# nrsyed/pytorch-yolov3

Hardware: AMD Instinct MI355X
Metric: frames/sec (608x608) (higher is better)
Workload: dtype bf16

## Files before the change

### pytorch-yolov3_amd/csrc/conv_fused.hip

```cpp
#include "common.h"
#include <type_traits>

namespace {

constexpr int kTO = 16;
constexpr int kSR = 2 * kTO + 1;
constexpr int kIR = kSR + 2;
constexpr int kInPitch = 144;
constexpr int kStemPitch = 80;
constexpr int kW1Pitch = 608;
constexpr int kNStem = kSR * kSR;
constexpr int kNFrag = (kNStem + 15) / 16;
constexpr int kThreads = 512;
constexpr int kInBytes = kIR * kInPitch * 2;
constexpr int kPatchElems = kIR * kIR * 3;
constexpr int kPre = (kPatchElems + kThreads - 1) / kThreads;
constexpr int kLds = 2 * kInBytes + kNStem * kStemPitch + 64 * kW1Pitch + 512;

template <typename T>
struct FusedArgs {
  const unsigned char *in;
  int H, W, batch;
  const T *w0;
  const float *sc0, *bi0;
  uint32_t flags0;
  const T *w1;
  int k_ld1;
  const float *sc1, *bi1;
  uint32_t flags1;
  T *out;
  int out_ld, Ho, Wo;
  int tiles_x, tiles_y, n_tiles;
  int dbg;
};

template <typename T>
__device__ __forceinline__ u32x2 bn_leaky_pack4(const f32x4 &a, const f32x4 &sc, const f32x4 &bi) {
  const f32x2 lo = f32x2{a[0], a[1]} * f32x2{sc[0], sc[1]} + f32x2{bi[0], bi[1]};
  const f32x2 hi = f32x2{a[2], a[3]} * f32x2{sc[2], sc[3]} + f32x2{bi[2], bi[3]};
  const f32x2 tl = lo * Y3_LEAKY_SLOPE, th = hi * Y3_LEAKY_SLOPE;
  return y3_pack4<T>(y3_vmax(lo[0], tl[0]), y3_vmax(lo[1], tl[1]), y3_vmax(hi[0], th[0]), y3_vmax(hi[1], th[1]));
}

template <typename T>
__global__ __launch_bounds__(kThreads) void conv_stem_s2_fused_kernel(FusedArgs<T> p) {
  typedef typename H16<T>::v8 V8;
  extern __shared__ __attribute__((aligned(16))) char smem[];
  T *in_tile = reinterpret_cast<T *>(smem);
  char *stem = smem + 2 * kInBytes;
  char *w1s = stem + kNStem * kStemPitch;
  T *lut = reinterpret_cast<T *>(w1s + 64 * kW1Pitch);

  const int tid = threadIdx.x, lane = tid & 63;
  const int wave = __builtin_amdgcn_readfirstlane(tid >> 6);
  const int fr = lane & 15, fq = lane >> 4;

  for (int i = tid; i < 64 * 36; i += kThreads) {
    const int co = i / 36, ch = i - co * 36;
    *reinterpret_cast<u32x4 *>(w1s + co * kW1Pitch + ch * 16) =
        *reinterpret_cast<const u32x4 *>(reinterpret_cast<const char *>(p.w1) + ((long long)co * p.k_ld1) * 2 + ch * 16);
  }
  V8 w0a[2], w0b[2];
#pragma unroll
  for (int st = 0; st < 2; ++st)
#pragma unroll
    for (int j = 0; j < 8; ++j) {
      const int k = st * 32 + fq * 8 + j;
      const int ky = k / 12, rem = k - ky * 12, kx = rem >> 2, c = rem & 3;
      const bool live = k < 36 && c < 3;
      const int kold = live ? ky * 9 + kx * 3 + c : 0;
      const T za = p.w0[(0 + fr) * 32 + kold], zb = p.w0[(16 + fr) * 32 + kold];
      w0a[st][j] = live ? za : (T)0.f;
      w0b[st][j] = live ? zb : (T)0.f;
    }
  int off_lo, off_hi;
  {
    const int k0 = fq * 8, k1 = fq * 8 + 4;
    off_lo = (k0 / 12) * kInPitch + (k0 % 12);
    off_hi = (k1 / 12) * kInPitch + (k1 % 12);
  }
  const int off_s1 = 2 * kInPitch + 8;
  const int cq = fq * 4;
  f32x4 sc0[2], bi0[2];
#pragma unroll
  for (int ni = 0; ni < 2; ++ni) {
    sc0[ni] = *reinterpret_cast<const f32x4 *>(p.sc0 + ni * 16 + cq);
    bi0[ni] = *reinterpret_cast<const f32x4 *>(p.bi0 + ni * 16 + cq);
  }

  int pr_row[kPre], pr_col[kPre], pr_dst[kPre];
  uint32_t pr_goff[kPre];
#pragma unroll
  for (int j = 0; j < kPre; ++j) {
    const int i = tid + j * kThreads;
    const int r = i / (kIR * 3), cb = i - r * (kIR * 3);
    pr_row[j] = r;
    pr_col[j] = cb;
    pr_goff[j] = (uint32_t)(r * p.W * 3 + cb);
    pr_dst[j] = r * kInPitch + (cb / 3) * 4 + (cb % 3);
  }
  const bool pr_last_live = tid + (kPre - 1) * kThreads < kPatchElems;
  auto tile_coords = [&](int tile, int &tx, int &ty, int &b) {
    int t = tile;
    tx = t % p.tiles_x;
    t /= p.tiles_x;
    ty = t % p.tiles_y;
    b = t / p.tiles_y;
  };
  auto patch_fetch = [&](int tile, unsigned char (&pre)[kPre]) {
    int tx, ty, b;
    tile_coords(tile, tx, ty, b);
    const int iy0 = 2 * ty * kTO - 2, ixb0 = (2 * tx * kTO - 2) * 3;
    const bool interior = iy0 >= 0 && iy0 + kIR <= p.H && ixb0 >= 0 && ixb0 + kIR * 3 <= p.W * 3;
    if (interior) {
      const unsigned char *base = p.in + ((long long)b * p.H + iy0) * p.W * 3 + ixb0;
#pragma unroll
      for (int j = 0; j < kPre; ++j) pre[j] = (j < kPre - 1 || pr_last_live) ? base[pr_goff[j]] : (unsigned char)0;
    } else {
#pragma unroll
      for (int j = 0; j < kPre; ++j) {
        const int iy = iy0 + pr_row[j], ixb = ixb0 + pr_col[j];
        unsigned char v = 0;
        if ((j < kPre - 1 || pr_last_live) && (unsigned)iy < (unsigned)p.H && ixb >= 0 && ixb < p.W * 3)
          v = p.in[((long long)b * p.H + iy) * p.W * 3 + ixb];
        pre[j] = v;
      }
    }
  };
  auto patch_store = [&](int buf, const unsigned char (&pre)[kPre]) {
    T *dst = in_tile + buf * (kIR * kInPitch);
#pragma unroll
    for (int j = 0; j < kPre; ++j)
      if (j < kPre - 1 || pr_last_live) dst[pr_dst[j]] = lut[pre[j]];
  };

  for (int i = tid; i < 2 * kIR * kInPitch / 2; i += kThreads) reinterpret_cast<uint32_t *>(in_tile)[i] = 0u;
  if (tid < 256) lut[tid] = (T)((float)tid / 255.0f);
  __syncthreads();
  int tile = blockIdx.x;
  int buf = 0;
  if (tile < p.n_tiles) {
    unsigned char pre[kPre];
    patch_fetch(tile, pre);
    patch_store(0, pre);
  }
  for (; tile < p.n_tiles; tile += gridDim.x) {
    int tx, ty, b;
    tile_coords(tile, tx, ty, b);
    const int oy0 = ty * kTO, ox0 = tx * kTO;
    __syncthreads();

    const T *patch = in_tile + buf * (kIR * kInPitch);
    const bool stem_inside = 2 * oy0 - 1 >= 0 && 2 * oy0 - 1 + kSR <= p.H && 2 * ox0 - 1 >= 0 && 2 * ox0 - 1 + kSR <= p.W;
    constexpr int kFG = 3;
    constexpr int kFragIters = (kNFrag + kThreads / 64 - 1) / (kThreads / 64);
    static_assert(kFragIters % kFG == 0, "fragment groups");
#pragma unroll 1
    for (int g = 0; g < ((p.dbg & 1) ? 0 : kFragIters); g += kFG) {
      u32x2 lo[kFG], hi[kFG], s1[kFG];
      int qv[kFG], syv[kFG], sxv[kFG];
#pragma unroll
      for (int j = 0; j < kFG; ++j) {
        const int q = (wave + (g + j) * (kThreads / 64)) * 16 + fr;
        const int qc = q < kNStem ? q : kNStem - 1;
        const int sy = qc / kSR, sx = qc - sy * kSR;
        const T *base = patch + sy * kInPitch + sx * 4;
        lo[j] = *reinterpret_cast<const u32x2 *>(base + off_lo);
        hi[j] = *reinterpret_cast<const u32x2 *>(base + off_hi);
        s1[j] = *reinterpret_cast<const u32x2 *>(base + off_s1);
        qv[j] = q;
        syv[j] = sy;
        sxv[j] = sx;
      }
      f32x4 acc0[kFG], acc1[kFG];
#pragma unroll
      for (int j = 0; j < kFG; ++j) {
        const V8 xf0 = __builtin_bit_cast(V8, u32x4{lo[j][0], lo[j][1], hi[j][0], hi[j][1]});
        acc0[j] = H16<T>::mfma(w0a[0], xf0, f32x4{0.f, 0.f, 0.f, 0.f});
        acc1[j] = H16<T>::mfma(w0b[0], xf0, f32x4{0.f, 0.f, 0.f, 0.f});
      }
#pragma unroll
      for (int j = 0; j < kFG; ++j) {
        const V8 xf1 = __builtin_bit_cast(V8, fq == 0 ? u32x4{s1[j][0], s1[j][1], 0u, 0u} : u32x4{0u, 0u, 0u, 0u});
        acc0[j] = H16<T>::mfma(w0a[1], xf1, acc0[j]);
        acc1[j] = H16<T>::mfma(w0b[1], xf1, acc1[j]);
      }
#pragma unroll
      for (int j = 0; j < kFG; ++j) {
        if (qv[j] < kNStem) {
          bool inside = true;
          if (!stem_inside) {
            const int gy = 2 * oy0 - 1 + syv[j], gx = 2 * ox0 - 1 + sxv[j];
            inside = (unsigned)gy < (unsigned)p.H && (unsigned)gx < (unsigned)p.W;
          }
#pragma unroll
          for (int ni = 0; ni < 2; ++ni) {
            u32x2 o = bn_leaky_pack4<T>(ni ? acc1[j] : acc0[j], sc0[ni], bi0[ni]);
            if (!inside) o = u32x2{0u, 0u};
            *reinterpret_cast<u32x2 *>(stem + qv[j] * kStemPitch + (ni * 16 + cq) * 2) = o;
          }
        }
      }
    }
    const int next_tile = tile + gridDim.x;
    unsigned char pre[kPre];
    if (next_tile < p.n_tiles && !(p.dbg & 8)) patch_fetch(next_tile, pre);
    __syncthreads();

    f32x4 acc[2][4];
#pragma unroll
    for (int mi = 0; mi < 2; ++mi)
#pragma unroll
      for (int nf = 0; nf < 4; ++nf) acc[mi][nf] = f32x4{0.f, 0.f, 0.f, 0.f};
#pragma unroll
    for (int tap = 0; tap < ((p.dbg & 2) ? 0 : 9); ++tap) {
      const int ky = tap / 3, kx = tap - ky * 3;
      u32x4 xf[2], wf[4];
#pragma unroll
      for (int mi = 0; mi < 2; ++mi) {
        const int q = (2 * (2 * wave + mi) + ky) * kSR + 2 * fr + kx;
        xf[mi] = *reinterpret_cast<const u32x4 *>(stem + q * kStemPitch + fq * 16);
      }
#pragma unroll
      for (int nf = 0; nf < 4; ++nf)
        wf[nf] = *reinterpret_cast<const u32x4 *>(w1s + (nf * 16 + fr) * kW1Pitch + tap * 64 + fq * 16);
#pragma unroll
      for (int mi = 0; mi < 2; ++mi)
#pragma unroll
        for (int nf = 0; nf < 4; ++nf)
          acc[mi][nf] = H16<T>::mfma(__builtin_bit_cast(V8, wf[nf]),
                                                                __builtin_bit_cast(V8, xf[mi]), acc[mi][nf]);
    }
    if (next_tile < p.n_tiles) patch_store(buf ^ 1, pre);
    __syncthreads();

#pragma unroll
    for (int nf = 0; nf < 4; ++nf) {
      const f32x4 s1 = *reinterpret_cast<const f32x4 *>(p.sc1 + nf * 16 + cq);
      const f32x4 b1 = *reinterpret_cast<const f32x4 *>(p.bi1 + nf * 16 + cq);
#pragma unroll
      for (int mi = 0; mi < 2; ++mi) {
        const int px = (2 * wave + mi) * kTO + fr;
        const int co = nf * 16 + cq;
        *reinterpret_cast<u32x2 *>(stem + px * 128 + (((co >> 3) ^ (px & 7)) << 4) + (co & 7) * 2) =
            bn_leaky_pack4<T>(acc[mi][nf], s1, b1);
      }
    }
    __syncthreads();
#pragma unroll
    for (int j = 0; j < kTO * kTO * 8 / kThreads; ++j) {
      const int i = tid + j * kThreads;
      const int px = i >> 3, ch = i & 7;
      const int oy = oy0 + (px >> 4), ox = ox0 + (px & 15);
      if (oy < p.Ho && ox < p.Wo && !(p.dbg & 4)) {
        const u32x4 v = *reinterpret_cast<const u32x4 *>(stem + px * 128 + ((ch ^ (px & 7)) << 4));
        *reinterpret_cast<u32x4 *>(p.out + (((long long)b * p.Ho + oy) * p.Wo + ox) * p.out_ld + ch * 8) = v;
      }
    }
    buf ^= 1;
  }
}


constexpr int kPX = 16, kPY = 8;
constexpr int kPSX = 2 * kPX + 1;
constexpr int kPSY = 2 * kPY + 1;
constexpr int kPIX = kPSX + 2, kPIY = kPSY + 2;
constexpr int kPNStem = kPSX * kPSY;
constexpr int kPNFrag = (kPNStem + 15) / 16;
constexpr int kPInBytes = kPIY * kInPitch * 2;
constexpr int kPStemBytes = kPNStem * kStemPitch;
constexpr int kPStage = 8 * 16 * 128;
constexpr int kPLds = 2 * kPInBytes + 2 * kPStemBytes + 64 * kW1Pitch + 512 + kPStage;
static_assert(kPLds <= 160 * 1024, "LDS budget");
static_assert(kPX == 16 && kPY == 8, "one 16-pixel output row per conv wave");

template <typename T, int NC>
__global__ __launch_bounds__(1024) void conv_stem_s2_ws_kernel(FusedArgs<T> p) {
  typedef typename H16<T>::v8 V8;
  constexpr int NS = 16 - NC, NT = 1024;
  constexpr int MR = kPY / NC;
  constexpr int kIters = (kPNFrag + NS - 1) / NS;
  constexpr int kPairs = kPIY * ((kPIX * 3 + 1) / 2);
  constexpr int kPre = (kPairs + 64 * NS - 1) / (64 * NS);
  extern __shared__ __attribute__((aligned(16))) char smem[];
  char *in_tile = smem;
  char *stem0 = smem + 2 * kPInBytes;
  char *w1s = stem0 + 2 * kPStemBytes;
  T *lut = reinterpret_cast<T *>(w1s + 64 * kW1Pitch);
  char *stage = reinterpret_cast<char *>(lut) + 512;

  const int tid = threadIdx.x, lane = tid & 63;
  const int wave = __builtin_amdgcn_readfirstlane(tid >> 6);
  const int fr = lane & 15, fq = lane >> 4;
  const bool is_stem = wave >= NC;

  for (int i = tid; i < 64 * 36; i += NT) {
    const int j = i / 36, ch = i - j * 36;
    const int co = y3_pair_perm(j);
    *reinterpret_cast<u32x4 *>(w1s + j * kW1Pitch + ch * 16) =
        *reinterpret_cast<const u32x4 *>(reinterpret_cast<const char *>(p.w1) + ((long long)co * p.k_ld1) * 2 + ch * 16);
  }
  for (int i = tid; i < 2 * kPInBytes / 4; i += NT) reinterpret_cast<uint32_t *>(in_tile)[i] = 0u;
  if (tid < 256) lut[tid] = (T)((float)tid / 255.0f);
  __syncthreads();
  const int tile0 = blockIdx.x, stride = gridDim.x;
  if (tile0 >= p.n_tiles) return;
  struct TilePos { int tile, tx, ty, b; };
  auto pos_of = [&](int tile) {
    TilePos t;
    t.tile = tile;
    t.tx = tile % p.tiles_x;
    const int r = tile / p.tiles_x;
    t.ty = r % p.tiles_y;
    t.b = r / p.tiles_y;
    return t;
  };
  const TilePos dpos = pos_of(stride);
  auto advance = [&](TilePos &t) {
    t.tile += stride;
    t.tx += dpos.tx;
    int c = t.tx >= p.tiles_x ? 1 : 0;
    t.tx -= c ? p.tiles_x : 0;
    t.ty += dpos.ty + c;
    c = t.ty >= p.tiles_y ? 1 : 0;
    t.ty -= c ? p.tiles_y : 0;
    t.b += dpos.b + c;
  };

  if (is_stem) {
    const int sw = wave - NC, stid = tid - 64 * NC;
    V8 w0a[2], w0b[2];
#pragma unroll
    for (int st = 0; st < 2; ++st)
#pragma unroll
      for (int j = 0; j < 8; ++j) {
        const int k = st * 32 + fq * 8 + j;
        const int ky = k / 12, rem = k - ky * 12, kx = rem >> 2, c = rem & 3;
        const bool live = k < 36 && c < 3;
        const int kold = live ? ky * 9 + kx * 3 + c : 0;
        const T za = p.w0[y3_pair_perm(fr) * 32 + kold], zb = p.w0[y3_pair_perm(16 + fr) * 32 + kold];
        w0a[st][j] = live ? za : (T)0.f;
        w0b[st][j] = live ? zb : (T)0.f;
      }
    int off_lo, off_hi;
    {
      const int k0 = fq * 8, k1 = fq * 8 + 4;
      off_lo = ((k0 / 12) * kInPitch + (k0 % 12)) * 2;
      off_hi = ((k1 / 12) * kInPitch + (k1 % 12)) * 2;
    }
    constexpr int off_s1 = (2 * kInPitch + 8) * 2;
    f32x4 sc0[2], bi0[2];
#pragma unroll
    for (int ni = 0; ni < 2; ++ni) {
      sc0[ni] = *reinterpret_cast<const f32x4 *>(p.sc0 + fq * 8 + ni * 4);
      bi0[ni] = *reinterpret_cast<const f32x4 *>(p.bi0 + fq * 8 + ni * 4);
    }
    int fr_patch[kIters];
    uint32_t fr_live = 0;
#pragma unroll
    for (int j = 0; j < kIters; ++j) {
      const int q = (sw + NS * j) * 16 + fr;
      const int qc = q < kPNStem ? q : kPNStem - 1;
      const int sy = qc / kPSX, sx = qc - sy * kPSX;
      fr_patch[j] = (sy * kInPitch + sx * 4) * 2;
      fr_live |= (q < kPNStem ? 1u : 0u) << j;
    }
    int stem_wr = ((sw * 16 + fr) * kStemPitch) + fq * 16;
    asm volatile("" : "+v"(stem_wr));
    constexpr int kRowPairs = (kPIX * 3 + 1) / 2;
    int pr_dst[kPre];
    uint32_t pr_goff[kPre];
    uint32_t pr_one = 0;
#pragma unroll
    for (int j = 0; j < kPre; ++j) {
      const int i = stid + j * 64 * NS;
      const int r = i / kRowPairs, cb = 2 * (i - r * kRowPairs);
      pr_goff[j] = (uint32_t)(r * p.W * 3 + cb);
      pr_dst[j] = (r * kInPitch + (cb / 3) * 4 + (cb % 3)) * 2 | (cb % 3 == 2 ? 1 : 0);
      pr_one |= (cb + 1 >= kPIX * 3 ? 1u : 0u) << j;
    }
    const bool pr_last_live = stid + (kPre - 1) * 64 * NS < kPairs;
    const bool pairs_aligned = ((p.W * 3) & 1) == 0 && (reinterpret_cast<size_t>(p.in) & 1) == 0;
    auto patch_fetch = [&](const TilePos &t, unsigned short (&pre)[kPre]) {
      const int tx = t.tx, ty = t.ty, b = t.b;
      const int iy0 = 2 * ty * kPY - 2, ixb0 = (2 * tx * kPX - 2) * 3;
      const bool interior = pairs_aligned && iy0 >= 0 && iy0 + kPIY <= p.H && ixb0 >= 0 && ixb0 + 2 * kRowPairs <= p.W * 3;
      if (interior) {
        const unsigned char *base = p.in + ((long long)b * p.H + iy0) * p.W * 3 + ixb0;
#pragma unroll
        for (int j = 0; j < kPre; ++j)
          pre[j] = (j < kPre - 1 || pr_last_live) ? *reinterpret_cast<const unsigned short *>(base + pr_goff[j]) : (unsigned short)0;
      } else {
#pragma unroll
        for (int j = 0; j < kPre; ++j) {
          const int i = stid + j * 64 * NS;
          const int r = i / kRowPairs, cb = 2 * (i - r * kRowPairs);
          const int iy = iy0 + r, ixb = ixb0 + cb;
          unsigned int v = 0;
          if ((j < kPre - 1 || pr_last_live) && (unsigned)iy < (unsigned)p.H) {
            const unsigned char *row = p.in + ((long long)b * p.H + iy) * p.W * 3;
            if (ixb >= 0 && ixb < p.W * 3) v = row[ixb];
            if (ixb + 1 >= 0 && ixb + 1 < p.W * 3 && cb + 1 < kPIX * 3) v |= (unsigned int)row[ixb + 1] << 8;
          }
          pre[j] = (unsigned short)v;
        }
      }
    };
    auto patch_store = [&](int buf, const unsigned short (&pre)[kPre]) {
      char *dst = in_tile + buf * kPInBytes;
#pragma unroll
      for (int j = 0; j < kPre; ++j)
        if (j < kPre - 1 || pr_last_live) {
          char *d = dst + (pr_dst[j] & ~1);
          *reinterpret_cast<T *>(d) = lut[pre[j] & 255];
          if (!((pr_one >> j) & 1u)) *reinterpret_cast<T *>(d + 2 + 2 * (pr_dst[j] & 1)) = lut[pre[j] >> 8];
        }
    };
    auto stem_image = [&](const char *patch, char *img, const TilePos &t) {
      const int oy0 = t.ty * kPY, ox0 = t.tx * kPX;
      const bool all_inside = 2 * oy0 - 1 >= 0 && 2 * oy0 - 1 + kPSY <= p.H && 2 * ox0 - 1 >= 0 && 2 * ox0 - 1 + kPSX <= p.W;
      auto group = [&](auto g0, auto cnt) {
        constexpr int g = decltype(g0)::value, G = decltype(cnt)::value;
        u32x2 lo[G], hi[G], s1[G];
#pragma unroll
        for (int j = 0; j < G; ++j) {
          const char *base = patch + fr_patch[g + j];
          lo[j] = *reinterpret_cast<const u32x2 *>(base + off_lo);
          hi[j] = *reinterpret_cast<const u32x2 *>(base + off_hi);
          s1[j] = *reinterpret_cast<const u32x2 *>(base + off_s1);
        }
        f32x4 a0[G], a1[G];
#pragma unroll
        for (int j = 0; j < G; ++j) {
          const V8 xf0 = __builtin_bit_cast(V8, u32x4{lo[j][0], lo[j][1], hi[j][0], hi[j][1]});
          a0[j] = H16<T>::mfma(w0a[0], xf0, f32x4{0.f, 0.f, 0.f, 0.f});
          a1[j] = H16<T>::mfma(w0b[0], xf0, f32x4{0.f, 0.f, 0.f, 0.f});
        }
#pragma unroll
        for (int j = 0; j < G; ++j) {
          const V8 xf1 = __builtin_bit_cast(V8, u32x4{s1[j][0], s1[j][1], s1[j][0], s1[j][1]});
          a0[j] = H16<T>::mfma(w0a[1], xf1, a0[j]);
          a1[j] = H16<T>::mfma(w0b[1], xf1, a1[j]);
        }
#pragma unroll
        for (int j = 0; j < G; ++j) {
          u32x2 o0 = bn_leaky_pack4<T>(a0[j], sc0[0], bi0[0]);
          u32x2 o1 = bn_leaky_pack4<T>(a1[j], sc0[1], bi0[1]);
          if (!all_inside) {
            const int q = (sw + NS * (g + j)) * 16 + fr;
            const int qc = q < kPNStem ? q : kPNStem - 1;
            const int sy = qc / kPSX, sx = qc - sy * kPSX;
            const int gy = 2 * oy0 - 1 + sy, gx = 2 * ox0 - 1 + sx;
            if (!((unsigned)gy < (unsigned)p.H && (unsigned)gx < (unsigned)p.W)) {
              o0 = u32x2{0u, 0u};
              o1 = u32x2{0u, 0u};
            }
          }
          if ((fr_live >> (g + j)) & 1u) {
            char *dst = img + stem_wr + (g + j) * (NS * 16 * kStemPitch);
            *reinterpret_cast<u32x4 *>(dst) = u32x4{o0[0], o0[1], o1[0], o1[1]};
          }
        }
      };
      using std::integral_constant;
      static_assert(kIters == 5 || kIters == 3, "fragment groups");
      group(integral_constant<int, 0>{}, integral_constant<int, 3>{});
      if constexpr (kIters == 5) group(integral_constant<int, 3>{}, integral_constant<int, 2>{});
    };

    unsigned short pre[4][kPre];
    TilePos fpos = pos_of(tile0);
    TilePos ipos = fpos;
    {
      patch_fetch(fpos, pre[0]);
      patch_store(0, pre[0]);
      advance(fpos);
      if (fpos.tile < p.n_tiles) {
        patch_fetch(fpos, pre[1]);
        patch_store(1, pre[1]);
      }
      advance(fpos);
    }
    __builtin_amdgcn_s_waitcnt(0xC07F);
    __builtin_amdgcn_s_barrier();
#pragma unroll
    for (int k = 0; k < 3; ++k) {
      if (fpos.tile < p.n_tiles) patch_fetch(fpos, pre[k]);
      advance(fpos);
    }
    stem_image(in_tile, stem0, ipos);
    advance(ipos);
    __builtin_amdgcn_s_waitcnt(0xC07F);
    __builtin_amdgcn_s_barrier();
    int par = 0;
    Y3_STAMP_DECL
    auto step = [&](auto setc) {
      constexpr int set = decltype(setc)::value;
      if (fpos.tile < p.n_tiles) patch_fetch(fpos, pre[(set + 3) & 3]);
      advance(fpos);
      Y3_STAMP(0);
      const bool more = ipos.tile < p.n_tiles;
      if (more) stem_image(in_tile + (par ^ 1) * kPInBytes, stem0 + (par ^ 1) * kPStemBytes, ipos);
      advance(ipos);
      __builtin_amdgcn_s_waitcnt(0xC07F);
      Y3_STAMP(1);
      if (ipos.tile < p.n_tiles) patch_store(par, pre[set]);
      __builtin_amdgcn_s_waitcnt(0xC07F);
      Y3_STAMP(2);
      __builtin_amdgcn_s_barrier();
      Y3_STAMP(3);
      par ^= 1;
      return more;
    };
    using std::integral_constant;
    for (;;) {
      if (!step(integral_constant<int, 0>{})) break;
      if (!step(integral_constant<int, 1>{})) break;
      if (!step(integral_constant<int, 2>{})) break;
      if (!step(integral_constant<int, 3>{})) break;
    }
#ifdef Y3_STAMPS
    if (tid == 64 * NC) for (int _i = 0; _i < 4; ++_i) atomicAdd(&g_y3_stamps[_i], _st_acc[_i]);
#endif
    return;
  }

  const int a_rd = ((2 * wave * MR) * kPSX + 2 * fr) * kStemPitch + fq * 16;
  const int b_rd = fr * kW1Pitch + fq * 16;
  char *my_stage = stage + wave * (MR * 16 * 128);
  f32x4 s1v[4], b1v[4];
#pragma unroll
  for (int nf = 0; nf < 4; ++nf) {
    s1v[nf] = *reinterpret_cast<const f32x4 *>(p.sc1 + (nf >> 1) * 32 + fq * 8 + (nf & 1) * 4);
    b1v[nf] = *reinterpret_cast<const f32x4 *>(p.bi1 + (nf >> 1) * 32 + fq * 8 + (nf & 1) * 4);
  }
  __builtin_amdgcn_s_waitcnt(0xC07F);
  __builtin_amdgcn_s_barrier();
  __builtin_amdgcn_s_barrier();
  uint32_t st_off[2];
#pragma unroll
  for (int k = 0; k < 2; ++k) st_off[k] = (uint32_t)((((lane >> 3) + 8 * k) * p.out_ld + (lane & 7) * 8) * 2);
  int par = 0;
  Y3_STAMP_DECL
  for (TilePos pos = pos_of(tile0); pos.tile < p.n_tiles; advance(pos)) {
    const int b = pos.b;
    const int oy0 = pos.ty * kPY, ox0 = pos.tx * kPX;
    const char *img = stem0 + par * kPStemBytes;
    f32x4 acc[MR][4];
#pragma unroll
    for (int mr = 0; mr < MR; ++mr)
#pragma unroll
      for (int nf = 0; nf < 4; ++nf) acc[mr][nf] = f32x4{0.f, 0.f, 0.f, 0.f};
#pragma unroll
    for (int tap = 0; tap < 9; ++tap) {
      const int ky = tap / 3, kx = tap - ky * 3;
      u32x4 xf[MR], wf[4];
#pragma unroll
      for (int mr = 0; mr < MR; ++mr)
        xf[mr] = *reinterpret_cast<const u32x4 *>(img + a_rd + ((2 * mr + ky) * kPSX + kx) * kStemPitch);
#pragma unroll
      for (int nf = 0; nf < 4; ++nf)
        wf[nf] = *reinterpret_cast<const u32x4 *>(w1s + b_rd + nf * 16 * kW1Pitch + tap * 64);
#pragma unroll
      for (int mr = 0; mr < MR; ++mr)
#pragma unroll
        for (int nf = 0; nf < 4; ++nf)
          acc[mr][nf] = H16<T>::mfma(__builtin_bit_cast(V8, wf[nf]),
                                                                __builtin_bit_cast(V8, xf[mr]), acc[mr][nf]);
    }
    Y3_STAMP(4);
#pragma unroll
    for (int mr = 0; mr < MR; ++mr)
#pragma unroll
      for (int k = 0; k < 2; ++k) {
        const u32x2 lo = bn_leaky_pack4<T>(acc[mr][2 * k], s1v[2 * k], b1v[2 * k]);
        const u32x2 hi = bn_leaky_pack4<T>(acc[mr][2 * k + 1], s1v[2 * k + 1], b1v[2 * k + 1]);
        *reinterpret_cast<u32x4 *>(my_stage + mr * 2048 + fr * 128 + (((k * 4 + fq) ^ (fr & 7)) << 4)) = u32x4{lo[0], lo[1], hi[0], hi[1]};
      }
    __builtin_amdgcn_wave_barrier();
#pragma unroll
    for (int mr = 0; mr < MR; ++mr) {
      const int oy = oy0 + wave * MR + mr;
      char *row = reinterpret_cast<char *>(p.out + (((long long)b * p.Ho + oy) * p.Wo + ox0) * p.out_ld);
      const bool full = ox0 + kPX <= p.Wo;
#pragma unroll
      for (int k = 0; k < 2; ++k) {
        const int px = (lane >> 3) + 8 * k, ch = lane & 7;
        const u32x4 v = *reinterpret_cast<const u32x4 *>(my_stage + mr * 2048 + px * 128 + ((ch ^ (px & 7)) << 4));
        if (oy < p.Ho && (full || ox0 + px < p.Wo)) *reinterpret_cast<u32x4 *>(row + st_off[k]) = v;
      }
    }
    __builtin_amdgcn_wave_barrier();
    __builtin_amdgcn_s_waitcnt(0xC07F);
    Y3_STAMP(5);
    __builtin_amdgcn_s_barrier();
    Y3_STAMP(6);
    par ^= 1;
  }
#ifdef Y3_STAMPS
  if (tid == 0) {
    for (int _i = 4; _i < 7; ++_i) atomicAdd(&g_y3_stamps[_i], _st_acc[_i]);
    atomicAdd(&g_y3_stamps[7], 1ull);
  }
#endif
}

constexpr int kRT = 16;
constexpr int kRP = kRT + 2;
constexpr int kRNP = kRP * kRP;
constexpr int kRFrag = (kRNP + 15) / 16;
constexpr int kYPitch = 96;
constexpr int kXBytes = kRNP * 128;
constexpr int kYBytes = 32768;
constexpr int kRLds = kXBytes + kYBytes + 64 * kW1Pitch;
constexpr int kXPre = (kRNP * 8 + kThreads - 1) / kThreads;
static_assert(kRNP * kYPitch <= kYBytes && kRT * kRT * 128 <= kYBytes, "image / staging tile must fit");

template <typename T>
struct ResArgs {
  const T *x;
  int H, W, batch, x_ld;
  const T *w2; int k_ld2; const float *sc2, *bi2;
  const T *w3; int k_ld3; const float *sc3, *bi3;
  T *out;
  int out_ld;
  int tiles_x, tiles_y, n_tiles;
};

template <typename T>
__global__ __launch_bounds__(kThreads) void conv_resblock_fused_kernel(ResArgs<T> p) {
  typedef typename H16<T>::v8 V8;
  extern __shared__ __attribute__((aligned(16))) char smem[];
  char *xt = smem;
  char *yt = smem + kXBytes;
  char *w3s = yt + kYBytes;

  const int tid = threadIdx.x, lane = tid & 63;
  const int wave = __builtin_amdgcn_readfirstlane(tid >> 6);
  const int fr = lane & 15, fq = lane >> 4;

  for (int i = tid; i < 64 * 36; i += kThreads) {
    const int j = i / 36, ch = i - j * 36;
    const int co = y3_pair_perm(j);
    *reinterpret_cast<u32x4 *>(w3s + j * kW1Pitch + ch * 16) =
        *reinterpret_cast<const u32x4 *>(reinterpret_cast<const char *>(p.w3) + ((long long)co * p.k_ld3) * 2 + ch * 16);
  }
  u32x4 w2f[2][2];
#pragma unroll
  for (int ni = 0; ni < 2; ++ni)
#pragma unroll
    for (int ks = 0; ks < 2; ++ks)
      w2f[ni][ks] = *reinterpret_cast<const u32x4 *>(reinterpret_cast<const char *>(p.w2) +
                                                    ((long long)y3_pair_perm(ni * 16 + fr) * p.k_ld2 + ks * 32 + fq * 8) * 2);
  f32x4 sc2[2], bi2[2];
#pragma unroll
  for (int ni = 0; ni < 2; ++ni) {
    sc2[ni] = *reinterpret_cast<const f32x4 *>(p.sc2 + fq * 8 + ni * 4);
    bi2[ni] = *reinterpret_cast<const f32x4 *>(p.bi2 + fq * 8 + ni * 4);
  }

  auto tile_origin = [&](int tile, int &b, int &oy0, int &ox0) {
    const int tx = tile % p.tiles_x;
    tile /= p.tiles_x;
    oy0 = (tile % p.tiles_y) * kRT;
    b = tile / p.tiles_y;
    ox0 = tx * kRT;
  };
  int xrc[kXPre];
  uint32_t xoff[kXPre];
  int xlds[kXPre];
#pragma unroll
  for (int j = 0; j < kXPre; ++j) {
    const int i = tid + j * kThreads;
    const int px = i >> 3, c = i & 7;
    const int r = px / kRP, cc = px - r * kRP;
    xrc[j] = i < kRNP * 8 ? (r << 8) | cc : -1;
    xoff[j] = ((uint32_t)(r * p.W + cc) * (uint32_t)p.x_ld) * 2u + (uint32_t)c * 16u;
    xlds[j] = px * 128 + ((c ^ (px & 7)) << 4);
  }
  constexpr int kAFr = (kRFrag + kThreads / 64 - 1) / (kThreads / 64);
  int a_rd[kAFr], a_rc[kAFr], a_wr[kAFr];
#pragma unroll
  for (int fs = 0; fs < kAFr; ++fs) {
    const int q = (wave + fs * (kThreads / 64)) * 16 + fr;
    const int qc = q < kRNP ? q : kRNP - 1;
    const int r = qc / kRP, cc = qc - r * kRP;
    a_rd[fs] = qc * 128 + ((fq ^ (qc & 7)) << 4);
    a_rc[fs] = (r << 8) | cc;
    a_wr[fs] = q < kRNP ? q * kYPitch + fq * 16 : -1;
  }
  constexpr int kOutPer = kRT * kRT * 8 / kThreads;
  int opx[kOutPer], olds[kOutPer];
  uint32_t ooff[kOutPer];
#pragma unroll
  for (int j = 0; j < kOutPer; ++j) {
    const int i = tid + j * kThreads;
    const int px = i >> 3, ch = i & 7;
    opx[j] = px;
    ooff[j] = ((uint32_t)((px >> 4) * p.W + (px & 15)) * (uint32_t)p.out_ld + (uint32_t)ch * 8u) * 2u;
    olds[j] = px * 128 + ((ch ^ (px & 7)) << 4);
  }
  auto x_fetch = [&](int tile, u32x4 (&pre)[kXPre]) {
    int b, oy0, ox0;
    tile_origin(tile, b, oy0, ox0);
    const char *base = reinterpret_cast<const char *>(p.x) + ((((long long)b * p.H + (oy0 - 1)) * p.W + (ox0 - 1)) * p.x_ld) * 2;
#pragma unroll
    for (int j = 0; j < kXPre; ++j) {
      const int gy = oy0 - 1 + (xrc[j] >> 8), gx = ox0 - 1 + (xrc[j] & 255);
      u32x4 v = {0u, 0u, 0u, 0u};
      if (xrc[j] >= 0 && (unsigned)gy < (unsigned)p.H && (unsigned)gx < (unsigned)p.W)
        v = *reinterpret_cast<const u32x4 *>(base + xoff[j]);
      pre[j] = v;
    }
  };
  auto x_store = [&](const u32x4 (&pre)[kXPre]) {
#pragma unroll
    for (int j = 0; j < kXPre; ++j)
      if (xrc[j] >= 0) *reinterpret_cast<u32x4 *>(xt + xlds[j]) = pre[j];
  };

  int tile = blockIdx.x;
  if (tile < p.n_tiles) {
    u32x4 pre[kXPre];
    x_fetch(tile, pre);
    x_store(pre);
  }
  for (; tile < p.n_tiles; tile += gridDim.x) {
    int b, oy0, ox0;
    tile_origin(tile, b, oy0, ox0);
    __syncthreads();

#pragma unroll
    for (int fs = 0; fs < kAFr; ++fs) {
      if (wave + fs * (kThreads / 64) >= kRFrag) break;
      const u32x4 xa = *reinterpret_cast<const u32x4 *>(xt + a_rd[fs]);
      const u32x4 xb = *reinterpret_cast<const u32x4 *>(xt + (a_rd[fs] ^ 64));
      const bool inside = (unsigned)(oy0 - 1 + (a_rc[fs] >> 8)) < (unsigned)p.H && (unsigned)(ox0 - 1 + (a_rc[fs] & 255)) < (unsigned)p.W;
      u32x2 o[2];
#pragma unroll
      for (int ni = 0; ni < 2; ++ni) {
        f32x4 a = {0.f, 0.f, 0.f, 0.f};
        a = H16<T>::mfma(__builtin_bit_cast(V8, w2f[ni][0]), __builtin_bit_cast(V8, xa), a);
        a = H16<T>::mfma(__builtin_bit_cast(V8, w2f[ni][1]), __builtin_bit_cast(V8, xb), a);
        o[ni] = bn_leaky_pack4<T>(a, sc2[ni], bi2[ni]);
        if (!inside) o[ni] = u32x2{0u, 0u};
      }
      if (a_wr[fs] >= 0) *reinterpret_cast<u32x4 *>(yt + a_wr[fs]) = u32x4{o[0][0], o[0][1], o[1][0], o[1][1]};
    }
    const int next_tile = tile + gridDim.x;
    u32x4 pre[kXPre];
    if (next_tile < p.n_tiles) x_fetch(next_tile, pre);
    __syncthreads();

    f32x4 acc[2][4];
#pragma unroll
    for (int mi = 0; mi < 2; ++mi)
#pragma unroll
      for (int nf = 0; nf < 4; ++nf) acc[mi][nf] = f32x4{0.f, 0.f, 0.f, 0.f};
#pragma unroll
    for (int tap = 0; tap < 9; ++tap) {
      const int ky = tap / 3, kx = tap - ky * 3;
      u32x4 xf[2], wf[4];
#pragma unroll
      for (int mi = 0; mi < 2; ++mi) {
        const int q = (2 * wave + mi + ky) * kRP + fr + kx;
        xf[mi] = *reinterpret_cast<const u32x4 *>(yt + q * kYPitch + fq * 16);
      }
#pragma unroll
      for (int nf = 0; nf < 4; ++nf)
        wf[nf] = *reinterpret_cast<const u32x4 *>(w3s + (nf * 16 + fr) * kW1Pitch + tap * 64 + fq * 16);
#pragma unroll
      for (int mi = 0; mi < 2; ++mi)
#pragma unroll
        for (int nf = 0; nf < 4; ++nf)
          acc[mi][nf] = H16<T>::mfma(__builtin_bit_cast(V8, wf[nf]),
                                                                __builtin_bit_cast(V8, xf[mi]), acc[mi][nf]);
    }
    __syncthreads();

#pragma unroll
    for (int k = 0; k < 2; ++k) {
      f32x4 s3[2], b3[2];
#pragma unroll
      for (int h = 0; h < 2; ++h) {
        s3[h] = *reinterpret_cast<const f32x4 *>(p.sc3 + k * 32 + fq * 8 + h * 4);
        b3[h] = *reinterpret_cast<const f32x4 *>(p.bi3 + k * 32 + fq * 8 + h * 4);
      }
#pragma unroll
      for (int mi = 0; mi < 2; ++mi) {
        const int oyl = 2 * wave + mi;
        const int pp = (oyl + 1) * kRP + fr + 1;
        const u32x4 xr = *reinterpret_cast<const u32x4 *>(xt + pp * 128 + (((k * 4 + fq) ^ (pp & 7)) << 4));
        float v[8];
        y3_bn_act8(v, acc[mi][2 * k], acc[mi][2 * k + 1], s3[0], s3[1], b3[0], b3[1], Y3_ACT_LEAKY);
        y3_add8<T>(v, xr);
        const int px = oyl * kRT + fr;
        *reinterpret_cast<u32x4 *>(yt + px * 128 + (((k * 4 + fq) ^ (px & 7)) << 4)) = y3_pack8<T>(v);
      }
    }
    __syncthreads();
    {
      char *obase = reinterpret_cast<char *>(p.out) + ((((long long)b * p.H + oy0) * p.W + ox0) * p.out_ld) * 2;
#pragma unroll
      for (int j = 0; j < kOutPer; ++j) {
        const int oy = oy0 + (opx[j] >> 4), ox = ox0 + (opx[j] & 15);
        if (oy < p.H && ox < p.W) *reinterpret_cast<u32x4 *>(obase + ooff[j]) = *reinterpret_cast<const u32x4 *>(yt + olds[j]);
      }
    }
    if (next_tile < p.n_tiles) x_store(pre);
  }
}

}


static int launch_stem_s2(const y3_op *ops, const y3_step &st, const void *d_in, const void *, hipStream_t s);
static int launch_resblock(const y3_op *ops, const y3_step &, const void *, const void *, hipStream_t s);

bool y3_choose_conv_fused_stem_s2(const y3_op &op0, const y3_op &op1, const y3_options &o, y3_step &st) {
  if (!o.fuse_stem) return false;
  if (!y3_conv_stem_mfma_supported(op0) || op0.out_c != 32 || (op0.flags & Y3_F_RESIDUAL)) return false;
  if (!(op0.flags & Y3_F_LEAKY) || !(op1.flags & Y3_F_LEAKY)) return false;
  if ((op0.flags | op1.flags) & Y3_F_MISH) return false;
  if (op1.kind != Y3_OP_CONV || op1.dtype != op0.dtype || op1.ksize != 3 || op1.stride != 2 || op1.pad != 1) return false;
  if (op1.in_c != 32 || op1.out_c != 64 || op1.out_ld % 8 != 0 || op1.out_ld < 64) return false;
  if (op1.flags & (Y3_F_RESIDUAL | Y3_F_OUT_F32 | Y3_F_IN_NCHW_F32 | Y3_F_IN_NHWC_U8BGR | Y3_F_PLAN_INPUT)) return false;
  if (op1.d_in != op0.d_out || op1.in_h != op0.out_h || op1.in_w != op0.out_w || op1.batch != op0.batch) return false;
  if (op1.k_ld < 288 || op1.cout_pad < 64) return false;
  if (op1.out_h != (op1.in_h + 2 - 3) / 2 + 1 || op1.out_w != (op1.in_w + 2 - 3) / 2 + 1) return false;
  st.launch = launch_stem_s2;
  st.name = op0.dtype == Y3_F16 ? "conv_stem_s2_fused_u8_f16" : "conv_stem_s2_fused_u8_bf16";
  st.pipelined = o.fuse_stem != 2;
  return true;
}

static int launch_stem_s2(const y3_op *ops, const y3_step &st, const void *d_in, const void *, hipStream_t s) {
  const y3_op &op0 = ops[0], &op1 = ops[1];
  return y3_by_dtype16(op0.dtype, [&](auto tag) {
    typedef decltype(tag) T;
    FusedArgs<T> a;
    a.in = static_cast<const unsigned char *>(d_in);
    a.H = op0.in_h; a.W = op0.in_w; a.batch = op0.batch;
    a.w0 = static_cast<const T *>(op0.d_weight);
    a.sc0 = op0.d_scale; a.bi0 = op0.d_bias; a.flags0 = op0.flags;
    a.w1 = static_cast<const T *>(op1.d_weight);
    a.k_ld1 = op1.k_ld;
    a.sc1 = op1.d_scale; a.bi1 = op1.d_bias; a.flags1 = op1.flags;
    a.out = static_cast<T *>(op1.d_out);
    a.out_ld = op1.out_ld; a.Ho = op1.out_h; a.Wo = op1.out_w;
    a.dbg = 0;
    static Y3DeviceOnce once;
    int n_cu = 0;
    {
      const int rc = once.run([]() -> int {
        Y3_HIP_CHECK(hipFuncSetAttribute(reinterpret_cast<const void *>(conv_stem_s2_fused_kernel<T>),
                                         hipFuncAttributeMaxDynamicSharedMemorySize, kLds));
        Y3_HIP_CHECK(hipFuncSetAttribute(reinterpret_cast<const void *>(conv_stem_s2_ws_kernel<T, 4>),
                                         hipFuncAttributeMaxDynamicSharedMemorySize, kPLds));
        return Y3_OK;
      }, &n_cu);
      if (rc != Y3_OK) return rc;
    }
    const bool pipelined = st.pipelined;
    a.tiles_x = y3_ceil_div(a.Wo, pipelined ? kPX : kTO);
    a.tiles_y = y3_ceil_div(a.Ho, pipelined ? kPY : kTO);
    a.n_tiles = a.tiles_x * a.tiles_y * a.batch;
    const int grid = a.n_tiles < n_cu ? a.n_tiles : n_cu;
    if (pipelined) Y3_LAUNCH((conv_stem_s2_ws_kernel<T, 4>), dim3(grid), dim3(1024), kPLds, s, a);
    else Y3_LAUNCH(conv_stem_s2_fused_kernel<T>, dim3(grid), dim3(kThreads), kLds, s, a);
    Y3_HIP_CHECK(hipGetLastError());
    return Y3_OK;
  });
}

bool y3_choose_conv_fused_resblock(const y3_op &op0, const y3_op &op1, const y3_options &o, y3_step &st) {
  if (!o.fuse_stem) return false;
  if (op0.kind != Y3_OP_CONV || op1.kind != Y3_OP_CONV || !y3_is16(op0.dtype) || op1.dtype != op0.dtype) return false;
  if (op0.ksize != 1 || op0.stride != 1 || op0.in_c != 64 || op0.out_c != 32) return false;
  if (op1.ksize != 3 || op1.stride != 1 || op1.pad != 1 || op1.in_c != 32 || op1.out_c != 64) return false;
  const uint32_t bad = Y3_F_OUT_F32 | Y3_F_IN_NCHW_F32 | Y3_F_IN_NHWC_U8BGR | Y3_F_PLAN_INPUT;
  if ((op0.flags & (bad | Y3_F_RESIDUAL)) || (op1.flags & bad)) return false;
  if (!(op0.flags & Y3_F_LEAKY) || !(op1.flags & Y3_F_LEAKY) || !(op1.flags & Y3_F_RESIDUAL)) return false;
  if ((op0.flags | op1.flags) & Y3_F_MISH) return false;
  if (op1.d_in != op0.d_out || op1.d_res != op0.d_in || op1.res_ld != op0.in_ld) return false;
  if (op0.in_h != op1.in_h || op0.in_w != op1.in_w || op0.batch != op1.batch) return false;
  if (op0.out_h != op0.in_h || op0.out_w != op0.in_w || op1.out_h != op1.in_h || op1.out_w != op1.in_w) return false;
  if (op0.in_ld % 8 != 0 || op1.out_ld % 8 != 0 || op0.in_ld < 64 || op1.out_ld < 64) return false;
  if (op0.k_ld < 64 || op1.k_ld < 288 || op0.cout_pad < 32 || op1.cout_pad < 64) return false;
  st.launch = launch_resblock;
  st.name = Y3_KNAME(op0.dtype, "conv_resblock_fused_", "_64_32_64");
  return true;
}

static int launch_resblock(const y3_op *ops, const y3_step &, const void *, const void *, hipStream_t s) {
  const y3_op &op0 = ops[0], &op1 = ops[1];
  return y3_by_dtype16(op0.dtype, [&](auto tag) {
    typedef decltype(tag) T;
    ResArgs<T> a;
    a.x = static_cast<const T *>(op0.d_in);
    a.H = op0.in_h; a.W = op0.in_w; a.batch = op0.batch; a.x_ld = op0.in_ld;
    a.w2 = static_cast<const T *>(op0.d_weight); a.k_ld2 = op0.k_ld; a.sc2 = op0.d_scale; a.bi2 = op0.d_bias;
    a.w3 = static_cast<const T *>(op1.d_weight); a.k_ld3 = op1.k_ld; a.sc3 = op1.d_scale; a.bi3 = op1.d_bias;
    a.out = static_cast<T *>(op1.d_out);
    a.out_ld = op1.out_ld;
    a.tiles_x = y3_ceil_div(a.W, kRT);
    a.tiles_y = y3_ceil_div(a.H, kRT);
    a.n_tiles = a.tiles_x * a.tiles_y * a.batch;
    static Y3DeviceOnce once;
    int n_cu = 0;
    {
      const int rc = once.run([]() -> int {
        Y3_HIP_CHECK(hipFuncSetAttribute(reinterpret_cast<const void *>(conv_resblock_fused_kernel<T>),
                                         hipFuncAttributeMaxDynamicSharedMemorySize, kRLds));
        return Y3_OK;
      }, &n_cu);
      if (rc != Y3_OK) return rc;
    }
    const int grid = a.n_tiles < n_cu ? a.n_tiles : n_cu;
    Y3_LAUNCH(conv_resblock_fused_kernel<T>, dim3(grid), dim3(kThreads), kRLds, s, a);
    Y3_HIP_CHECK(hipGetLastError());
    return Y3_OK;
  });
}

Y3_STAMP_READER(y3_debug_stamps_fused)
```

Measured before the change: 5884.

## Add warp-specialized pipelined fused resblock kernel with producer/consumer waves

Adds a 1024-thread resblock kernel in which 12 producer waves fetch input tiles from global memory and compute the 1x1 conv into LDS, while 4 consumer waves run the 3x3 conv, residual add and store. Input tiles are triple-buffered and the intermediate is double-buffered, so loads and the 1x1 stage overlap the 3x3 stage. Tiles shrink to 16x8. The goal is to hide global memory latency and stage serialization. It costs more LDS, smaller tiles with more halo overhead, and barrier-coupled scheduling between waves. It becomes the default path unless fuse_stem==2.

```diff
diff --git a/pytorch-yolov3_amd/csrc/conv_fused.hip b/pytorch-yolov3_amd/csrc/conv_fused.hip
--- a/pytorch-yolov3_amd/csrc/conv_fused.hip
+++ b/pytorch-yolov3_amd/csrc/conv_fused.hip
@@ -812,6 +812,263 @@
   }
 }
 
+constexpr int kQX = 16, kQY = 8;
+constexpr int kQPX = kQX + 2, kQPY = kQY + 2;
+constexpr int kQNP = kQPX * kQPY;
+constexpr int kQFrag = (kQNP + 15) / 16;
+constexpr int kQXBytes = kQNP * 128;
+constexpr int kQYBytes = kQNP * kYPitch;
+constexpr int kQLds = 3 * kQXBytes + 2 * kQYBytes + 64 * kW1Pitch + 512;
+static_assert(kQLds <= 160 * 1024, "LDS budget");
+
+struct TileCursor { int tile, tx, ty, b; };
+__device__ __forceinline__ TileCursor tile_cursor(int tile, int tiles_x, int tiles_y) {
+  TileCursor t;
+  t.tile = tile;
+  t.tx = tile % tiles_x;
+  const int r = tile / tiles_x;
+  t.ty = r % tiles_y;
+  t.b = r / tiles_y;
+  return t;
+}
+__device__ __forceinline__ void tile_advance(TileCursor &t, const TileCursor &d, int tiles_x, int tiles_y) {
+  t.tile += d.tile;
+  t.tx += d.tx;
+  int c = t.tx >= tiles_x ? 1 : 0;
+  t.tx -= c ? tiles_x : 0;
+  t.ty += d.ty + c;
+  c = t.ty >= tiles_y ? 1 : 0;
+  t.ty -= c ? tiles_y : 0;
+  t.b += d.b + c;
+}
+
+template <typename T, int NC>
+__global__ __launch_bounds__(1024) void conv_resblock_ws_kernel(ResArgs<T> p) {
+  typedef typename H16<T>::v8 V8;
+  constexpr int NS = 16 - NC, MR = kQY / NC;
+  constexpr int kAF = (kQFrag + NS - 1) / NS;
+  constexpr int kPre = (kQNP * 8 + 64 * NS - 1) / (64 * NS);
+  static_assert(kQY % NC == 0, "whole output rows per conv wave");
+  extern __shared__ __attribute__((aligned(16))) char smem[];
+  char *xt0 = smem;
+  char *yt0 = smem + 3 * kQXBytes;
+  char *w3s = yt0 + 2 * kQYBytes;
+  float *sb3 = reinterpret_cast<float *>(w3s + 64 * kW1Pitch);
+
+  const int tid = threadIdx.x, lane = tid & 63;
+  const int wave = __builtin_amdgcn_readfirstlane(tid >> 6);
+  const int fr = lane & 15, fq = lane >> 4;
+
+  if (tid < 128) sb3[tid] = tid < 64 ? p.sc3[tid] : p.bi3[tid - 64];
+  for (int i = tid; i < 64 * 36; i += 1024) {
+    const int j = i / 36, ch = i - j * 36;
+    const int co = y3_pair_perm(j);
+    *reinterpret_cast<u32x4 *>(w3s + j * kW1Pitch + ch * 16) =
+        *reinterpret_cast<const u32x4 *>(reinterpret_cast<const char *>(p.w3) + ((long long)co * p.k_ld3) * 2 + ch * 16);
+  }
+  const int tile0 = blockIdx.x;
+  if (tile0 >= p.n_tiles) return;
+  const TileCursor dpos = tile_cursor(gridDim.x, p.tiles_x, p.tiles_y);
+  auto advance = [&](TileCursor &t) { tile_advance(t, dpos, p.tiles_x, p.tiles_y); };
+
+  if (wave >= NC) {
+    const int sw = wave - NC, stid = tid - 64 * NC;
+    u32x4 w2f[2][2];
+#pragma unroll
+    for (int ni = 0; ni < 2; ++ni)
+#pragma unroll
+      for (int ks = 0; ks < 2; ++ks)
+        w2f[ni][ks] = *reinterpret_cast<const u32x4 *>(reinterpret_cast<const char *>(p.w2) +
+                                                      ((long long)y3_pair_perm(ni * 16 + fr) * p.k_ld2 + ks * 32 + fq * 8) * 2);
+    f32x4 sc2[2], bi2[2];
+#pragma unroll
+    for (int ni = 0; ni < 2; ++ni) {
+      sc2[ni] = *reinterpret_cast<const f32x4 *>(p.sc2 + fq * 8 + ni * 4);
+      bi2[ni] = *reinterpret_cast<const f32x4 *>(p.bi2 + fq * 8 + ni * 4);
+    }
+    int xrc[kPre];
+    uint32_t xoff[kPre];
+    int xlds[kPre];
+#pragma unroll
+    for (int j = 0; j < kPre; ++j) {
+      const int i = stid + j * 64 * NS;
+      const int px = i >> 3, c = i & 7;
+      const int r = px / kQPX, cc = px - r * kQPX;
+      xrc[j] = i < kQNP * 8 ? (r << 8) | cc : -1;
+      xoff[j] = ((uint32_t)(r * p.W + cc) * (uint32_t)p.x_ld) * 2u + (uint32_t)c * 16u;
+      xlds[j] = px * 128 + ((c ^ (px & 7)) << 4);
+    }
+    int a_rd[kAF], a_rc[kAF], a_wr[kAF];
+#pragma unroll
+    for (int fs = 0; fs < kAF; ++fs) {
+      const int q = (sw + NS * fs) * 16 + fr;
+      const int qc = q < kQNP ? q : kQNP - 1;
+      const int r = qc / kQPX, cc = qc - r * kQPX;
+      a_rd[fs] = qc * 128 + ((fq ^ (qc & 7)) << 4);
+      a_rc[fs] = (r << 8) | cc;
+      a_wr[fs] = q < kQNP ? q * kYPitch + fq * 16 : -1;
+    }
+    auto x_fetch = [&](const TileCursor &t, u32x4 (&pre)[kPre], uint32_t &live) {
+      const int oy0 = t.ty * kQY, ox0 = t.tx * kQX;
+      const bool tile_ok = t.tile < p.n_tiles;
+      const char *base = reinterpret_cast<const char *>(p.x) + ((((long long)t.b * p.H + (oy0 - 1)) * p.W + (ox0 - 1)) * p.x_ld) * 2;
+      live = 0;
+#pragma unroll
+      for (int j = 0; j < kPre; ++j) {
+        const int gy = oy0 - 1 + (xrc[j] >> 8), gx = ox0 - 1 + (xrc[j] & 255);
+        const bool ok = tile_ok && xrc[j] >= 0 && (unsigned)gy < (unsigned)p.H && (unsigned)gx < (unsigned)p.W;
+        const char *src = ok ? base + xoff[j] : reinterpret_cast<const char *>(p.x);
+        pre[j] = *reinterpret_cast<const u32x4 *>(src);
+        live |= (ok ? 1u : 0u) << j;
+      }
+    };
+    auto x_store = [&](char *xt, const u32x4 (&pre)[kPre], uint32_t live) {
+#pragma unroll
+      for (int j = 0; j < kPre; ++j)
+        if (xrc[j] >= 0) *reinterpret_cast<u32x4 *>(xt + xlds[j]) = ((live >> j) & 1u) ? pre[j] : u32x4{0u, 0u, 0u, 0u};
+    };
+    auto image = [&](const char *xt, char *yt, const TileCursor &t) {
+      const int oy0 = t.ty * kQY, ox0 = t.tx * kQX;
+#pragma unroll
+      for (int fs = 0; fs < kAF; ++fs) {
+        if (sw + NS * fs >= kQFrag) break;
+        const u32x4 xa = *reinterpret_cast<const u32x4 *>(xt + a_rd[fs]);
+        const u32x4 xb = *reinterpret_cast<const u32x4 *>(xt + (a_rd[fs] ^ 64));
+        const bool inside = (unsigned)(oy0 - 1 + (a_rc[fs] >> 8)) < (unsigned)p.H && (unsigned)(ox0 - 1 + (a_rc[fs] & 255)) < (unsigned)p.W;
+        u32x2 o[2];
+#pragma unroll
+        for (int ni = 0; ni < 2; ++ni) {
+          f32x4 a = {0.f, 0.f, 0.f, 0.f};
+          a = H16<T>::mfma(__builtin_bit_cast(V8, w2f[ni][0]), __builtin_bit_cast(V8, xa), a);
+          a = H16<T>::mfma(__builtin_bit_cast(V8, w2f[ni][1]), __builtin_bit_cast(V8, xb), a);
+          o[ni] = bn_leaky_pack4<T>(a, sc2[ni], bi2[ni]);
+          if (!inside) o[ni] = u32x2{0u, 0u};
+        }
+        if (a_wr[fs] >= 0) *reinterpret_cast<u32x4 *>(yt + a_wr[fs]) = u32x4{o[0][0], o[0][1], o[1][0], o[1][1]};
+      }
+    };
+
+    u32x4 pre[4][kPre];
+    uint32_t live[4];
+    TileCursor fpos = tile_cursor(tile0, p.tiles_x, p.tiles_y);
+    TileCursor ipos = fpos;
+    x_fetch(fpos, pre[0], live[0]);
+    x_store(xt0, pre[0], live[0]);
+    advance(fpos);
+    x_fetch(fpos, pre[1], live[1]);
+    x_store(xt0 + kQXBytes, pre[1], live[1]);
+    advance(fpos);
+    __builtin_amdgcn_s_waitcnt(0xC07F);
+    __builtin_amdgcn_s_barrier();
+#pragma unroll
+    for (int k = 0; k < 3; ++k) {
+      x_fetch(fpos, pre[k], live[k]);
+      advance(fpos);
+    }
+    image(xt0, yt0, ipos);
+    advance(ipos);
+    __builtin_amdgcn_s_waitcnt(0xC07F);
+    __builtin_amdgcn_s_barrier();
+    int par = 0, xb = 0;
+    auto step = [&](auto setc) {
+      constexpr int set = decltype(setc)::value;
+      x_fetch(fpos, pre[(set + 3) & 3], live[(set + 3) & 3]);
+      advance(fpos);
+      const int x1 = xb == 2 ? 0 : xb + 1, x2 = x1 == 2 ? 0 : x1 + 1;
+      const bool more = ipos.tile < p.n_tiles;
+      if (more) image(xt0 + x1 * kQXBytes, yt0 + (par ^ 1) * kQYBytes, ipos);
+      advance(ipos);
+      if (ipos.tile < p.n_tiles) x_store(xt0 + x2 * kQXBytes, pre[set], live[set]);
+      __builtin_amdgcn_s_waitcnt(0xC07F);
+      __builtin_amdgcn_s_barrier();
+      par ^= 1;
+      xb = x1;
+      return more;
+    };
+    using std::integral_constant;
+    for (;;) {
+      if (!step(integral_constant<int, 0>{})) break;
+      if (!step(integral_constant<int, 1>{})) break;
+      if (!step(integral_constant<int, 2>{})) break;
+      if (!step(integral_constant<int, 3>{})) break;
+    }
+    return;
+  }
+
+  const int a_rd = ((wave * MR) * kQPX + fr) * kYPitch + fq * 16;
+  const int b_rd = fr * kW1Pitch + fq * 16;
+  __builtin_amdgcn_s_waitcnt(0xC07F);
+  __builtin_amdgcn_s_barrier();
+  __builtin_amdgcn_s_barrier();
+  uint32_t st_off[2];
+#pragma unroll
+  for (int k = 0; k < 2; ++k) st_off[k] = (uint32_t)((((lane >> 3) + 8 * k) * p.out_ld + (lane & 7) * 8) * 2);
+  int par = 0, xb = 0;
+  for (TileCursor pos = tile_cursor(tile0, p.tiles_x, p.tiles_y); pos.tile < p.n_tiles; advance(pos)) {
+    const int oy0 = pos.ty * kQY, ox0 = pos.tx * kQX;
+    const char *img = yt0 + par * kQYBytes;
+    char *xt = xt0 + xb * kQXBytes;
+    f32x4 acc[MR][4];
+#pragma unroll
+    for (int mr = 0; mr < MR; ++mr)
+#pragma unroll
+      for (int nf = 0; nf < 4; ++nf) acc[mr][nf] = f32x4{0.f, 0.f, 0.f, 0.f};
+#pragma unroll
+    for (int tap = 0; tap < 9; ++tap) {
+      const int ky = tap / 3, kx = tap - ky * 3;
+      u32x4 xf[MR], wf[4];
+#pragma unroll
+      for (int mr = 0; mr < MR; ++mr)
+        xf[mr] = *reinterpret_cast<const u32x4 *>(img + a_rd + ((mr + ky) * kQPX + kx) * kYPitch);
+#pragma unroll
+      for (int nf = 0; nf < 4; ++nf)
+        wf[nf] = *reinterpret_cast<const u32x4 *>(w3s + b_rd + nf * 16 * kW1Pitch + tap * 64);
+#pragma unroll
+      for (int mr = 0; mr < MR; ++mr)
+#pragma unroll
+        for (int nf = 0; nf < 4; ++nf)
+          acc[mr][nf] = H16<T>::mfma(__builtin_bit_cast(V8, wf[nf]), __builtin_bit_cast(V8, xf[mr]), acc[mr][nf]);
+    }
+    f32x4 s3v[4], b3v[4];
+#pragma unroll
+    for (int nf = 0; nf < 4; ++nf) {
+      s3v[nf] = *reinterpret_cast<const f32x4 *>(sb3 + (nf >> 1) * 32 + fq * 8 + (nf & 1) * 4);
+      b3v[nf] = *reinterpret_cast<const f32x4 *>(sb3 + 64 + (nf >> 1) * 32 + fq * 8 + (nf & 1) * 4);
+    }
+#pragma unroll
+    for (int mr = 0; mr < MR; ++mr)
+#pragma unroll
+      for (int k = 0; k < 2; ++k) {
+        const int pp = (wave * MR + mr + 1) * kQPX + fr + 1;
+        u32x4 *xp = reinterpret_cast<u32x4 *>(xt + pp * 128 + (((k * 4 + fq) ^ (pp & 7)) << 4));
+        const u32x4 xr = *xp;
+        float v[8];
+        y3_bn_act8(v, acc[mr][2 * k], acc[mr][2 * k + 1], s3v[2 * k], s3v[2 * k + 1], b3v[2 * k], b3v[2 * k + 1], Y3_ACT_LEAKY);
+        y3_add8<T>(v, xr);
+        *xp = y3_pack8<T>(v);
+      }
+    __builtin_amdgcn_wave_barrier();
+    const bool full = ox0 + kQX <= p.W;
+#pragma unroll
+    for (int mr = 0; mr < MR; ++mr) {
+      const int oy = oy0 + wave * MR + mr;
+      char *row = reinterpret_cast<char *>(p.out) + ((((long long)pos.b * p.H + oy) * p.W + ox0) * p.out_ld) * 2;
+#pragma unroll
+      for (int k = 0; k < 2; ++k) {
+        const int px = (lane >> 3) + 8 * k, ch = lane & 7;
+        const int pp = (wave * MR + mr + 1) * kQPX + px + 1;
+        const u32x4 v = *reinterpret_cast<const u32x4 *>(xt + pp * 128 + ((ch ^ (pp & 7)) << 4));
+        if (oy < p.H && (full || ox0 + px < p.W)) *reinterpret_cast<u32x4 *>(row + st_off[k]) = v;
+      }
+    }
+    __builtin_amdgcn_wave_barrier();
+    __builtin_amdgcn_s_waitcnt(0xC07F);
+    __builtin_amdgcn_s_barrier();
+    par ^= 1;
+    xb = xb == 2 ? 0 : xb + 1;
+  }
+}
+
 }
 
 
@@ -890,10 +1147,13 @@
   if (op0.k_ld < 64 || op1.k_ld < 288 || op0.cout_pad < 32 || op1.cout_pad < 64) return false;
   st.launch = launch_resblock;
   st.name = Y3_KNAME(op0.dtype, "conv_resblock_fused_", "_64_32_64");
+  st.pipelined = o.fuse_stem != 2;
   return true;
 }
 
-static int launch_resblock(const y3_op *ops, const y3_step &, const void *, const void *, hipStream_t s) {
+constexpr int kResNC = 4;
+
+static int launch_resblock(const y3_op *ops, const y3_step &st, const void *, const void *, hipStream_t s) {
   const y3_op &op0 = ops[0], &op1 = ops[1];
   return y3_by_dtype16(op0.dtype, [&](auto tag) {
     typedef decltype(tag) T;
@@ -904,8 +1164,9 @@
     a.w3 = static_cast<const T *>(op1.d_weight); a.k_ld3 = op1.k_ld; a.sc3 = op1.d_scale; a.bi3 = op1.d_bias;
     a.out = static_cast<T *>(op1.d_out);
     a.out_ld = op1.out_ld;
-    a.tiles_x = y3_ceil_div(a.W, kRT);
-    a.tiles_y = y3_ceil_div(a.H, kRT);
+    const bool pipelined = st.pipelined;
+    a.tiles_x = y3_ceil_div(a.W, pipelined ? kQX : kRT);
+    a.tiles_y = y3_ceil_div(a.H, pipelined ? kQY : kRT);
     a.n_tiles = a.tiles_x * a.tiles_y * a.batch;
     static Y3DeviceOnce once;
     int n_cu = 0;
@@ -913,12 +1174,15 @@
       const int rc = once.run([]() -> int {
         Y3_HIP_CHECK(hipFuncSetAttribute(reinterpret_cast<const void *>(conv_resblock_fused_kernel<T>),
                                          hipFuncAttributeMaxDynamicSharedMemorySize, kRLds));
+        Y3_HIP_CHECK(hipFuncSetAttribute(reinterpret_cast<const void *>(conv_resblock_ws_kernel<T, kResNC>),
+                                         hipFuncAttributeMaxDynamicSharedMemorySize, kQLds));
         return Y3_OK;
       }, &n_cu);
       if (rc != Y3_OK) return rc;
     }
     const int grid = a.n_tiles < n_cu ? a.n_tiles : n_cu;
-    Y3_LAUNCH(conv_resblock_fused_kernel<T>, dim3(grid), dim3(kThreads), kRLds, s, a);
+    if (pipelined) Y3_LAUNCH((conv_resblock_ws_kernel<T, kResNC>), dim3(grid), dim3(1024), kQLds, s, a);
+    else Y3_LAUNCH(conv_resblock_fused_kernel<T>, dim3(grid), dim3(kThreads), kRLds, s, a);
     Y3_HIP_CHECK(hipGetLastError());
     return Y3_OK;
   });
```

Result: no change. 5892, median of 6 (+0.1%).
